# IK2277/ultimate-tictactoe-alphazero

Measured on NVIDIA B200. Metric: self-play moves/sec (50 sims/move), higher is better.
Workload: dtype bf16

## Files before the change

### ultimate-tictactoe-alphazero_b200/csrc/common.cuh

```cuda
#pragma once
#include <cuda_bf16.h>
#include <cuda_runtime.h>
#include <stdint.h>
#include <stdio.h>

#include "../../include/uttt_b200.h"
#include "uttt_rules.cuh"

namespace uttt {

void set_error(const char* fmt, ...);

#define UTTT_CUDA_OK(expr)                                                                   \
    do {                                                                                     \
        cudaError_t _e = (expr);                                                             \
        if (_e != cudaSuccess) {                                                             \
            ::uttt::set_error("%s failed: %s (%s:%d)", #expr, cudaGetErrorString(_e), __FILE__, __LINE__); \
            return 1;                                                                        \
        }                                                                                    \
    } while (0)

#define UTTT_CHECK(cond, ...)               \
    do {                                    \
        if (!(cond)) {                      \
            ::uttt::set_error(__VA_ARGS__); \
            return 2;                       \
        }                                   \
    } while (0)

static inline int ceil_div(int64_t a, int64_t b) { return (int)((a + b - 1) / b); }

#ifdef __CUDACC__
__device__ __forceinline__ void pdl_wait() { asm volatile("griddepcontrol.wait;" ::: "memory"); }
__device__ __forceinline__ void pdl_trigger() { asm volatile("griddepcontrol.launch_dependents;" ::: "memory"); }
template <typename... KArgs, typename... Args>
cudaError_t launch_pdl(void (*kernel)(KArgs...), dim3 grid, dim3 block, size_t smem, cudaStream_t s, Args... args) {
    cudaLaunchConfig_t cfg = {};
    cfg.gridDim = grid; cfg.blockDim = block; cfg.dynamicSmemBytes = smem; cfg.stream = s;
    cudaLaunchAttribute attr[1];
    attr[0].id = cudaLaunchAttributeProgrammaticStreamSerialization;
    attr[0].val.programmaticStreamSerializationAllowed = 1;
    cfg.attrs = attr; cfg.numAttrs = 1;
    return cudaLaunchKernelEx(&cfg, kernel, KArgs(args)...);
}
#endif

constexpr int NET_C = 128;
constexpr int NET_BLOCKS = 16;
constexpr int NET_LAYERS = 2 * NET_BLOCKS;
// ... 43 lines not shown
    const float* value;
    int32_t row_stride, copy_stride;
    int32_t* out_counts;
    int32_t* out_n;
    uint32_t seed;
    uint64_t game0;
    int64_t n_games;
    unsigned long long* counters;
    PackedState* hist_states;
    uint16_t* hist_counts;
    uint8_t* hist_actions;
    int32_t* hist_len;
    int8_t* hist_final;
    uint8_t* slot_flags;
    unsigned long long* dbg_tree;
};

cudaError_t launch_tree_begin(const TreeParams& p, cudaStream_t s);
cudaError_t launch_tree_round(const TreeParams& p, cudaStream_t s);
cudaError_t launch_tree_tp_begin(const TreeParams& p, cudaStream_t s);
cudaError_t launch_tree_tp_round(const TreeParams& p, cudaStream_t s);
cudaError_t launch_hash_eval(const PackedState* states, const int32_t* k, const int32_t* count, int max_rows,
                             float* policy, float* value, int row_stride, int copy_stride, cudaStream_t s);
cudaError_t launch_scores(const int32_t* counts, const int32_t* n, int n_trees, float temperature,
                          float* scores, cudaStream_t s);
cudaError_t launch_dirichlet(uint32_t seed, uint64_t game0, int64_t n, int n_children, float alpha, float* out, cudaStream_t s);
cudaError_t launch_boltzman(const float* xs, int n, float temperature, float* out, cudaStream_t s);

cudaError_t launch_scan_lens(const int32_t* lens, int64_t n, int64_t* offsets, cudaStream_t s);
cudaError_t launch_pack_samples(const PackedState* states, const uint16_t* counts, const int32_t* lens, const int8_t* final_lose,
                                const int64_t* offsets, int64_t n_games, void* out, int64_t cap_samples, cudaStream_t s);
cudaError_t launch_unpack_samples(const void* samples, int64_t n, float* x, float* policy, float* value, cudaStream_t s);

// ... 34 lines not shown
                              float* out, cudaStream_t s);
cudaError_t launch_trunk_fp32(const NetWeights& w, const __nv_bfloat16* planes, const int32_t* count, int max_rows,
                              float* act_a, float* act_b, cudaStream_t s);
cudaError_t launch_heads_fc(const NetWeights& w, const float* headfeat, const int32_t* count, int max_rows, float* policy,
                            float* value, int row_stride, cudaStream_t s);
cudaError_t launch_heads(const NetWeights& w, const float* act_f32, const __nv_bfloat16* act_bf16,
                         const int32_t* count, int max_rows, float* policy, float* value, int row_stride,
                         cudaStream_t s);
cudaError_t launch_trunk_x3(const NetWeights& w, const __nv_bfloat16* planes, float* headfeat, const int32_t* count,
                            int max_rows, float* skip, int n_sm, cudaStream_t s, long long* dbg);
int trunk_pp_cap1(int n_sm);
cudaError_t launch_trunk_pp_large(const NetWeights& w, const __nv_bfloat16* planes, float* headfeat, const int32_t* count,
                                  int max_rows, float* skip, int n_sm, cudaStream_t s, long long* dbg);
cudaError_t launch_trunk_auto(const NetWeights& w, const __nv_bfloat16* planes, float* headfeat, const int32_t* count, int max_rows,
                              float* skip, int n_sm, cudaStream_t s, long long* dbg, float* policy, float* value,
                              const uint8_t* slot_flags = nullptr, int n_slots = 0);

}
```

### ultimate-tictactoe-alphazero_b200/csrc/engine.cu

```cuda
#include <math.h>
#include <stdlib.h>
#include <string.h>

#include <vector>

#include "common.cuh"

using namespace uttt;

namespace {

constexpr int CHECK_EVERY = 8;
constexpr int N_LANES = 2;
constexpr int N_WINDOWS = 2;
constexpr int EV_POOL = N_WINDOWS * CHECK_EVERY * 4 * N_LANES;

__global__ void set_int_kernel(int32_t* p, int32_t v) { *p = v; }
__global__ void set_u64_kernel(unsigned long long* p, unsigned long long v) { *p = v; }

template <typename T>
cudaError_t dmalloc(T** p, size_t n) { return cudaMalloc((void**)p, n * sizeof(T)); }

}

// ... 94 lines not shown
    bool heads_fused = false;
    if (evaluator == UTTT_EVAL_NET_FP32) {
        if (ev3) cudaEventRecord(ev3[0], s);
        UTTT_CUDA_OK(launch_trunk_fp32(e->w, b.nn_planes, count, max_rows, b.act_a, b.act_b, s));
        e->prof_launches[1] += 1 + 2 * NET_BLOCKS;
    } else if (evaluator == UTTT_EVAL_NET_BF16X3) {
        if (ev3) cudaEventRecord(ev3[0], s);
        UTTT_CUDA_OK(launch_trunk_x3(e->w, b.nn_planes, b.headfeat, count, max_rows, b.resid, e->n_sm, s, e->tc_dbg));
        e->prof_launches[1] += 1;
    } else if (evaluator == UTTT_EVAL_NET_BF16) {
        if (ev3) cudaEventRecord(ev3[0], s);
        heads_fused = max_rows <= trunk_pp_cap1(e->n_sm);
        UTTT_CHECK(heads_fused || !b.slot_flags, "slot mode needs the fused heads");
        UTTT_CUDA_OK(launch_trunk_auto(e->w, b.nn_planes, b.headfeat, count, max_rows, b.resid, e->n_sm, s, e->tc_dbg,
                                       heads_fused ? b.policy : nullptr, heads_fused ? b.value : nullptr, b.slot_flags,
                                       b.n_slots));
        if (!heads_fused)
            UTTT_CUDA_OK(launch_trunk_pp_large(e->w, b.nn_planes, b.headfeat, count, max_rows, b.resid, e->n_sm, s, e->tc_dbg));
        e->prof_launches[1] += 1;
    } else {
        UTTT_CHECK(false, "evaluator %d cannot run on the device", evaluator);
    }
    if (ev3) cudaEventRecord(ev3[1], s);
    if (heads_fused) {
        if (ev3 && e->prof_level >= 2) cudaEventRecord(ev3[2], s);
        return 0;
    }
    if (evaluator == UTTT_EVAL_NET_BF16 || evaluator == UTTT_EVAL_NET_BF16X3)
        UTTT_CUDA_OK(launch_heads_fc(e->w, b.headfeat, count, max_rows, b.policy, b.value, 1, s));
    else
        UTTT_CUDA_OK(launch_heads(e->w, b.act_a, nullptr, count, max_rows, b.policy, b.value, 1, s));
// ... 69 lines not shown
    uttt_engine* e = new uttt_engine();
    memset(&e->tp, 0, sizeof(e->tp));
    memset(&e->w, 0, sizeof(e->w));
    e->cfg = *cfg;
    e->trace_on = false;
    e->progress_cb = nullptr;
    e->progress_user = nullptr;
    e->prof_level = getenv("UTTT_PROFILE") ? atoi(getenv("UTTT_PROFILE")) : 1;
    e->prof_sample = getenv("UTTT_PROFILE_SAMPLE") ? atoi(getenv("UTTT_PROFILE_SAMPLE")) : 4;
    if (e->prof_sample < 1) e->prof_sample = 1;
    e->lane_threshold = getenv("UTTT_LANE_THRESHOLD") ? atoi(getenv("UTTT_LANE_THRESHOLD")) : 1024;
    UTTT_CUDA_OK(net_fp32_init());
    UTTT_CUDA_OK(trunk_tc2_init());
    UTTT_CUDA_OK(trunk_pp_init());
    UTTT_CUDA_OK(trunk_auto_init());
    cudaDeviceProp prop;
    UTTT_CUDA_OK(cudaGetDeviceProperties(&prop, cfg->device));
    e->n_sm = prop.multiProcessorCount;
    e->node_cap = 1 + 81 + 81 * cfg->max_sims;
    e->rows_per_slot = cfg->max_batch < TP_MAX_LEAVES ? cfg->max_batch : TP_MAX_LEAVES;
    UTTT_CUDA_OK(cudaStreamCreateWithFlags(&e->stream, cudaStreamNonBlocking));
    size_t S = (size_t)cfg->n_slots, NC = (size_t)e->node_cap, G = (size_t)cfg->max_games;
    size_t R = S * (size_t)e->rows_per_slot;
    TreeParams& t = e->tp;
    t.node_cap = e->node_cap;
    if (ealloc(e, &t.root, S) || ealloc(e, &t.leaf_state, S * TP_MAX_LEAVES) ||
        ealloc(e, &t.tp_paths, S * TP_MAX_LEAVES * PATH_CAP) || ealloc(e, &t.tp_aux, S * 2 * TP_MAX_LEAVES) || ealloc(e, &t.ctl, S) ||
        ealloc(e, &t.path, S * PATH_CAP) || ealloc(e, &t.nodes, S * NC) ||
        ealloc(e, &t.nn_states, R) || ealloc(e, &t.nn_planes, R * 243 + 8) || ealloc(e, &t.nn_tree, R) ||
        ealloc(e, &t.nn_k, R) || ealloc(e, &t.nn_count, 2 * N_LANES) || ealloc(e, &t.out_counts, S * 81) ||
// ... 16 lines not shown
        for (int w = 0; w < N_WINDOWS; w++) UTTT_CUDA_OK(cudaEventCreateWithFlags(&e->ev_win[w][i], cudaEventDisableTiming));
    }
    UTTT_CUDA_OK(cudaEventCreateWithFlags(&e->ev_fork, cudaEventDisableTiming));
    UTTT_CUDA_OK(cudaEventCreateWithFlags(&e->ev_fwd, cudaEventDisableTiming));
    UTTT_CUDA_OK(cudaEventCreateWithFlags(&e->ev_idle, cudaEventDisableTiming));
    e->fwd_pending = false;
    UTTT_CUDA_OK(cudaMallocHost((void**)&e->h_counters, 8 * (1 + N_WINDOWS) * sizeof(unsigned long long)));
    UTTT_CUDA_OK(cudaMallocHost((void**)&e->h_count, 2 * sizeof(int32_t)));
    for (int i = 0; i < EV_POOL; i++) UTTT_CUDA_OK(cudaEventCreate(&e->ev[i]));
    t.policy = e->policy;
    t.value = e->value;
    t.dbg_tree = nullptr;
    if (getenv("UTTT_DEBUG_TREE")) {
        if (ealloc(e, &t.dbg_tree, 48)) { uttt_destroy(e); return 1; }
        UTTT_CUDA_OK(cudaMemset(t.dbg_tree, 0, 48 * sizeof(unsigned long long)));
    }
    t.max_terminal = getenv("UTTT_MAX_TERMINAL") ? atoi(getenv("UTTT_MAX_TERMINAL")) : 4;
    t.dir_alpha = 0.3f;
    t.dir_eps = 0.25f;
    t.temperature = 1.0f;
    *out = e;
    return 0;
}

int uttt_destroy(uttt_engine* e) {
    if (!e) return 0;
    cudaSetDevice(e->cfg.device);
    cudaDeviceSynchronize();
    for (void* p : e->allocs) cudaFree(p);
    release_weights(e->w);
// ... 450 lines not shown
                0ll, d[1] - d[0], d[2] - d[0], d[3] - d[0], d[4] - d[0], d[5] - d[0], d[6] - d[0], d[8] - d[0], d[9] - d[0], d[10] - d[0], d[11] - d[0],
                d[12] - d[0], d[13] - d[0], d[14] - d[0]);
        fprintf(stderr, "tc2 detail, layer 20 -> 21 (cycles rel. accumulator observed by epilogue thread 0): last MMA of layer 20 committed %lld | "
                "first chunk loaded %lld, stored %lld, fenced %lld, chunks published %lld %lld %lld %lld | issuer of tile 0 passed the "
                "act barrier of quarter 0..3 at %lld %lld %lld %lld\n", d[12] - d[0], d[1] - d[0], d[2] - d[0], d[3] - d[0], d[4] - d[0],
                d[5] - d[0], d[6] - d[0], d[7] - d[0], d[8] - d[0], d[9] - d[0], d[10] - d[0], d[11] - d[0]);
        long long au[10];
        UTTT_CUDA_OK(cudaMemcpy(au, e->tc_dbg + 200, sizeof(au), cudaMemcpyDeviceToHost));
        fprintf(stderr, "heads FC tail (cycles rel. body done): barriers ready %lld, features loaded %lld, chunk 0/1/2 landed %lld %lld %lld, "
                "policy FC done %lld, all FC done %lld, exit %lld\n", au[3] - au[1], au[4] - au[1], au[5] - au[1], au[6] - au[1],
                au[7] - au[1], au[8] - au[1], au[9] - au[1], au[2] - au[1]);
        fprintf(stderr, "trunk_auto_kernel CTA 0 (cycles rel. entry): body done %lld, heads FC done %lld (warp 0's exit; heads = %lld)\n",
                au[1] - au[0], au[2] - au[0], au[2] - au[1]);
        fprintf(stderr, "trunk phases (cycles rel. entry): setup %lld, first MMA %lld, last epilogue %lld, exit %lld\n", ph[1] - ph[0],
                (long long)out128[0] - ph[0], ph[2] - ph[0], ph[3] - ph[0]);
    }
    return 0;
}

int uttt_debug_batch_histogram(uttt_engine* e, int64_t* out64, int32_t reset) {
    UTTT_CHECK(e && out64, "null argument");
    UTTT_CUDA_OK(cudaSetDevice(e->cfg.device));
    UTTT_CUDA_OK(cudaDeviceSynchronize());
    UTTT_CUDA_OK(cudaMemcpy(out64, e->tc_dbg + 128, 64 * sizeof(long long), cudaMemcpyDeviceToHost));
    if (reset) UTTT_CUDA_OK(cudaMemset(e->tc_dbg + 128, 0, 64 * sizeof(long long)));
    return 0;
}

int uttt_debug_trace(uttt_engine* e, int enable) {
    UTTT_CHECK(e != nullptr, "null engine");
// ... 51 lines not shown
```

### ultimate-tictactoe-alphazero_b200/csrc/net_auto.cu

```cuda
#include "heads_fc.cuh"
#include "net_pp_kernel.cuh"
#include "net_tc2_kernel.cuh"

namespace uttt {

static_assert(tc2::Cfg<>::THREADS == pp::THREADS, "one block size for both bodies");
constexpr int AUTO_SMEM = tc2::Cfg<>::SMEM_BYTES > pp::Cfg<1>::SMEM_BYTES ? tc2::Cfg<>::SMEM_BYTES : pp::Cfg<1>::SMEM_BYTES;
static_assert(HEADS_SMEM_BYTES <= AUTO_SMEM, "the fused heads reuse the trunk's shared memory");

constexpr int SLOT_CHUNKS = 17;
__device__ __forceinline__ void scan_slots(const uint8_t* __restrict__ flags, int n_slots, int n_pairs, int pair, int small_cap,
                                           int* s_npos, int* s_src) {
    const int lane = threadIdx.x & 31;
    uint32_t mine = 0;
#pragma unroll
    for (int j = 0; j < SLOT_CHUNKS; j++) {
        const int idx = lane + 32 * j;
        if (idx < n_slots && flags[idx]) mine |= 1u << j;
    }
    uint32_t bal[SLOT_CHUNKS];
    int n_pos = 0;
#pragma unroll
    for (int j = 0; j < SLOT_CHUNKS; j++) {
        bal[j] = __ballot_sync(0xFFFFFFFFu, (mine >> j) & 1u);
// ... 2 lines not shown
    const int P = n_pos <= small_cap ? tc2::group_positions(n_pos, n_pairs) : pp::pair_positions<1>(n_pos, n_pairs);
    const int first = pair * P, last = min(n_pos, first + P);
    int run = 0;
#pragma unroll
    for (int j = 0; j < SLOT_CHUNKS; j++) {
        if ((bal[j] >> lane) & 1u) {
            const int rank = run + __popc(bal[j] & ((1u << lane) - 1u));
            if (rank >= first && rank < last) s_src[rank - first] = lane + 32 * j;
        }
        run += __popc(bal[j]);
    }
    if (lane == 0) *s_npos = n_pos;
}

constexpr int AUTO_SMEM_TOTAL = AUTO_SMEM + 64;

__global__ void __cluster_dims__(2, 1, 1) __launch_bounds__(pp::THREADS, 1)
trunk_auto_kernel(const __nv_bfloat16* __restrict__ res_w8, const __nv_bfloat16* __restrict__ conv_in_w8,
                  const __nv_bfloat16* __restrict__ res_w18, const __nv_bfloat16* __restrict__ conv_in_w18,
                  const __nv_bfloat16* __restrict__ bias_2sm,
                  const __nv_bfloat16* __restrict__ planes, const float* __restrict__ headw, float* headfeat, uint4* skip,
                  const int32_t* __restrict__ count, int small_cap, int cap1, long long* dbg,
                  HeadsFC fc, float* policy, float* value ,
                  const uint8_t* __restrict__ slot_flags, int n_slots ) {
    extern __shared__ __align__(1024) uint8_t smem[];
    pdl_trigger();
    pdl_wait();
    const bool stamp = dbg && blockIdx.x == 0 && threadIdx.x == 0;
    if (stamp) dbg[200] = clock64();
    const int n_pairs = (int)gridDim.x >> 1, pair = (int)blockIdx.x >> 1;
    int* s_src = reinterpret_cast<int*>(smem + AUTO_SMEM);
    int* s_npos = s_src + 8;
    int n_pos;
    if (slot_flags) {
        if (threadIdx.x < 32) scan_slots(slot_flags, n_slots, n_pairs, pair, small_cap, s_npos, s_src);
        __syncthreads();
        n_pos = *s_npos;
    } else {
        n_pos = *count;
    }
    const int* src = slot_flags ? s_src : nullptr;
    const bool small = n_pos <= small_cap;
    if (n_pos <= 0 || n_pos > cap1) return;
    tcx::count_batch(dbg, n_pos);
    if (!small)
        pp::trunk_pp_body<1>(res_w18, conv_in_w18, bias_2sm, planes, headw, headfeat, skip, dbg, n_pos, src);
    else
        tc2::trunk_tc2_body<false>(res_w8, conv_in_w8, bias_2sm, planes, headw, headfeat, skip, dbg, n_pos, src, 0, false);
    if (stamp) dbg[201] = clock64();
    if (policy == nullptr) return;
    const int P = small ? tc2::group_positions(n_pos, n_pairs) : pp::pair_positions<1>(n_pos, n_pairs);
    const int first = pair * P, last = min(n_pos, first + P);
    const int rank = (int)tcx::cluster_rank();
    const int row0 = first + rank;
    const int np = row0 < last ? (last - row0 + 1) >> 1 : 0;
    static_assert((pp::Cfg<1>::MAX_PA + pp::Cfg<1>::MAX_PB + 1) / 2 <= HEADS_P, "one heads call per CTA");
    if (np == 0) return;
    heads_fc_block(fc, headfeat, row0, 2, np, policy, value, 1, reinterpret_cast<float*>(smem), stamp ? dbg + 203 : nullptr,
                   src ? src + rank : nullptr);
    if (stamp) dbg[202] = clock64();
}

cudaError_t trunk_auto_init() {
    return cudaFuncSetAttribute(trunk_auto_kernel, cudaFuncAttributeMaxDynamicSharedMemorySize, AUTO_SMEM_TOTAL);
}

cudaError_t launch_trunk_auto(const NetWeights& w, const __nv_bfloat16* planes, float* headfeat, const int32_t* count, int max_rows,
                              float* skip, int n_sm, cudaStream_t s, long long* dbg, float* policy, float* value,
                              const uint8_t* slot_flags, int n_slots) {
    int pairs = n_sm / 2;
    if (max_rows < pairs) pairs = max_rows < 1 ? 1 : max_rows;
    const int small_cap = (n_sm / 2) * tc2::Cfg<>::MAX_P;
    const int cap1 = (n_sm / 2) * (pp::Cfg<1>::MAX_PA + pp::Cfg<1>::MAX_PB);
    if (policy && max_rows > cap1) return cudaErrorInvalidValue;
    if (slot_flags && (!policy || n_slots > 32 * SLOT_CHUNKS || n_slots > max_rows)) return cudaErrorInvalidValue;
    return launch_pdl(trunk_auto_kernel, dim3(2 * pairs), dim3(pp::THREADS), AUTO_SMEM_TOTAL, s, w.res_w_2sm, w.conv_in_w_2sm,
                      w.res_w_2sm18, w.conv_in_w_2sm18, w.bias_blk_2sm, planes, w.head_w, headfeat, reinterpret_cast<uint4*>(skip),
                      count, small_cap, cap1, dbg, heads_fc_of(w), policy, value, slot_flags, n_slots);
}

}
```

### ultimate-tictactoe-alphazero_b200/csrc/net_pp_kernel.cuh

```cuda
#pragma once
#include "tc_common.cuh"

namespace uttt {
namespace pp {

using namespace tcx;

constexpr int POS_ROWS = 100;
constexpr int LEAD = 11;
constexpr int LT = 2;
constexpr int NG = 2;
constexpr int BIAS_BYTES = 2048;
constexpr int CONST_BYTES = 4096;
constexpr int EPI_WARPS = 8 * LT;
constexpr int THREADS = (EPI_WARPS + 1 + LT) * 32;
constexpr int SKIP_ROWS = 128 * LT;
constexpr int GROUP_LAYERS = NET_LAYERS + 1;
constexpr uint32_t IDESC = IDESC_M256_N128_BF16;
constexpr int a_rows(int tiles) { return (LEAD + 128 * tiles + 11 + 7) / 8 * 8; }

template <int LTB>
struct Cfg {
    static constexpr int MAX_PA = 5, MAX_PB = (LTB == 1) ? 2 : 5;
    static constexpr int PANEL_A = a_rows(LT) * 16, PANEL_B = a_rows(LTB) * 16;
// ... 37 lines not shown
__host__ __device__ inline int pair_positions(int n_pos, int n_pairs) {
    int P = (n_pos + n_pairs - 1) / n_pairs;
    return P < 1 ? 1 : (P > Cfg<LTB>::MAX_PA + Cfg<LTB>::MAX_PB ? Cfg<LTB>::MAX_PA + Cfg<LTB>::MAX_PB : P);
}

template <int LTB>
__device__ __forceinline__ void trunk_pp_body(const __nv_bfloat16* __restrict__ wq,
                const __nv_bfloat16* __restrict__ wq_in,
                const __nv_bfloat16* __restrict__ wq_bias,
                const __nv_bfloat16* __restrict__ planes,
                const float* __restrict__ headw,
                float* headfeat,
                uint4* skip,
                long long* dbg,
                int n_pos,
                const int* src_rows) {
    using C = Cfg<LTB>;
    constexpr int STAGES = C::STAGES, BAR_OFF = C::BAR_OFF, HEAD_OFF = C::HEAD_OFF, CONST_OFF = C::CONST_OFF,
                  STAGE_BLOCKS = C::STAGE_BLOCKS, STAGE_BYTES = C::STAGE_BYTES, STAGES_PER_LAYER = C::STAGES_PER_LAYER,
                  IN_STAGES = C::IN_STAGES;
    constexpr int MAX_P = C::MAX_PA;
    extern __shared__ __align__(1024) uint8_t smem[];
    const int warp = threadIdx.x >> 5, lane = threadIdx.x & 31;
    const uint32_t rank = cluster_rank();
    const uint32_t peer = rank ^ 1u;
    const int n_pairs = (int)gridDim.x >> 1, pair = (int)blockIdx.x >> 1;
    const int Ptot = pair_positions<LTB>(n_pos, n_pairs);
    const int n_super = (n_pos + Ptot - 1) / Ptot;
    if (pair >= n_super) return;
    const int PA = Ptot < MAX_P ? Ptot : MAX_P;
    const Geo geo[NG] = {make_geo(PA, rank), make_geo(Ptot - PA, rank)};
    const bool any_tiles = geo[0].T0 + geo[1].T0 > 0;

    uint8_t* sA = smem;
    const uint32_t sA_u = smem_u32(sA);
    const uint32_t sB_u = sA_u + C::W_OFF;
    auto grp_off = [](int g) { return (uint32_t)(g == 0 ? 0 : C::A_BYTES); };
    auto grp_panel = [](int g) { return (uint32_t)(g == 0 ? C::PANEL_A : C::PANEL_B); };
    const uint32_t bar_u = sA_u + BAR_OFF;
    const uint32_t bar_full = bar_u, bar_empty = bar_u + 8 * STAGES, bar_grp = bar_u + 16 * STAGES;
    constexpr int GRP_BARS = 2 * LT;
    auto bar_accum = [&](int g, int t) { return bar_grp + 8u * (uint32_t)(g * GRP_BARS + t); };
    auto bar_act = [&](int g, int t) { return bar_grp + 8u * (uint32_t)(g * GRP_BARS + LT + t); };
    static_assert(16 * STAGES + 8 * NG * GRP_BARS + 4 <= 512, "barrier block");
    uint32_t* tmem_holder = reinterpret_cast<uint32_t*>(smem + BAR_OFF + 16 * STAGES + 8 * NG * GRP_BARS);
    const int bnd_quarter = (rank == 0) ? 3 : 0;

    if (threadIdx.x == 0) {
        for (int i = 0; i < STAGES; i++) {
            mbar_init(bar_full + 8 * i, rank == 0 ? 2 : 1);
            mbar_init(bar_empty + 8 * i, LT);
        }
        for (int g = 0; g < NG; g++) {
            for (int t = 0; t < LT; t++) {
                mbar_init(bar_accum(g, t), 1);
                mbar_init(bar_act(g, t), 8 + (t > 0 ? 2 : 0) + (t < geo[g].tiles - 1 ? 2 : 0) + ((rank == 0 && t < geo[g].T1) ? 1 : 0));
            }
        }
        asm volatile("fence.mbarrier_init.release.cluster;" ::: "memory");
    }
    if (warp == EPI_WARPS + 1) {
        asm volatile("tcgen05.alloc.cta_group::2.sync.aligned.shared::cta.b32 [%0], %1;" ::"r"(smem_u32(tmem_holder)), "r"(512u)
                     : "memory");
        asm volatile("tcgen05.relinquish_alloc_permit.cta_group::2.sync.aligned;" ::: "memory");
    }
    for (int i = threadIdx.x; i < (C::A_BYTES + C::B_BYTES) / 16; i += THREADS) reinterpret_cast<uint4*>(sA)[i] = make_uint4(0, 0, 0, 0);
    for (int i = threadIdx.x; i < CONST_BYTES / 16; i += THREADS)
        reinterpret_cast<uint4*>(sA + CONST_OFF)[i] = (i < 128) ? make_uint4(0x3F803F80u, 0, 0, 0) : make_uint4(0, 0, 0, 0);
    fence_async_smem();
    tc_fence_before();
    __syncthreads();
    cluster_sync_all();
    tc_fence_after();
    const uint32_t tmem_base = *tmem_holder;

    int iter = 0;
    for (int sg = pair; sg < n_super; sg += n_pairs, iter++) {
        if (warp < EPI_WARPS) {
            const int lt = warp >> 3, quarter = warp & 3, chalf = (warp >> 2) & 1;
            const int lr = lt * 128 + quarter * 32 + lane;
            const uint4 zero4 = make_uint4(0, 0, 0, 0);
// ... 301 lines not shown
                                    if (dbg && blockIdx.x == 0 && iter == 0 && lt == 0 && layer < 16) dbg[(16 * g + layer) * 4 + 1] = clock64();
                                }
                            }
                            advance();
                        }
                    }
                }
            }
            __syncwarp();
        }
    }

    tc_fence_before();
    __syncthreads();
    cluster_sync_all();
    if (warp == EPI_WARPS + 1) {
        asm volatile("tcgen05.dealloc.cta_group::2.sync.aligned.b32 %0, %1;" ::"r"(tmem_base), "r"(512u) : "memory");
    }
}

}
}
```

### ultimate-tictactoe-alphazero_b200/csrc/net_tc2_kernel.cuh

```cuda
#pragma once
#include <stdlib.h>

#include "tc_common.cuh"


namespace uttt {
namespace tc2 {

constexpr int POS_ROWS = 100;
constexpr int LEAD = 11;
constexpr int GROUP_LAYERS = NET_LAYERS + 1;

template <bool X3 = false>
struct Cfg {
    static constexpr int LOC_TILES = 2;
    static constexpr int MAX_P = 5;
    static constexpr int AROWS = (LEAD + 128 * LOC_TILES + 11 + 7) / 8 * 8;
    static constexpr int PANEL_BYTES = AROWS * 16;
    static constexpr int ACT_PANELS = X3 ? 32 : 16;
    static constexpr int A_BYTES = (ACT_PANELS + 2) * PANEL_BYTES;
    static constexpr int STAGES = X3 ? 3 : 8;
    static constexpr int STAGE_BLOCKS = X3 ? 6 : 8;
    static constexpr int NCO = 64;
    static constexpr int SUB_BYTES = 2 * NCO * 16;
// ... 24 lines not shown
    if (P == 4) P = 5;
    return P;
}

template <bool X3>
__device__ __forceinline__ void trunk_tc2_body(const __nv_bfloat16* __restrict__ wq,
                 const __nv_bfloat16* __restrict__ wq_in,
                 const __nv_bfloat16* __restrict__ wq_bias,
                 const __nv_bfloat16* __restrict__ planes,
                 const float* __restrict__ headw,
                 float* headfeat,
                 uint4* skip,
                 long long* dbg,
                 int n_pos,
                 const int* src_rows,
                 int pos_base, bool solo) {
    using C = Cfg<X3>;
    constexpr int LOC_TILES = C::LOC_TILES, PANEL_BYTES = C::PANEL_BYTES, A_BYTES = C::A_BYTES,
                  STAGES = C::STAGES, BAR_OFF = C::BAR_OFF, EPI_WARPS = C::EPI_WARPS, THREADS = C::THREADS,
                  SKIP_ROWS = C::SKIP_ROWS, NQ = C::NQ, STAGE_BLOCKS = C::STAGE_BLOCKS, STAGE_BYTES = C::STAGE_BYTES,
                  STAGES_PER_LAYER = C::STAGES_PER_LAYER, IN_STAGES = C::IN_STAGES, GROUP_STAGES = C::GROUP_STAGES,
                  ACT_PANELS = C::ACT_PANELS, SKIP_U4 = C::SKIP_U4, BLOCK_BYTES = C::BLOCK_BYTES;
    extern __shared__ __align__(1024) uint8_t smem[];
    const long long t_entry = clock64();
    const int warp = threadIdx.x >> 5, lane = threadIdx.x & 31;
    const uint32_t rank = cluster_rank();
    const int n_pairs = solo ? 1 : (int)gridDim.x >> 1, pair = solo ? 0 : (int)blockIdx.x >> 1;
    const int P = group_positions(n_pos, n_pairs);
    const int T = (P * POS_ROWS + 127) / 128;
    const int T0 = (T + 1) >> 1;
    const int tiles = (rank == 0) ? T0 : T - T0;
    const int tile0 = (rank == 0) ? 0 : T0;
    const int n_groups = (n_pos + P - 1) / P;
    if (pair >= n_groups) return;
    const int T1 = T - T0;
    const bool has_peer = T1 > 0;

    uint8_t* sA = smem;
    const uint32_t sA_u = smem_u32(sA);
    const uint32_t sB_u = sA_u + A_BYTES;
    const uint32_t bar_u = sA_u + BAR_OFF;
    const uint32_t bar_full = bar_u, bar_empty = bar_u + 8 * STAGES, bar_accum = bar_u + 16 * STAGES,
                   bar_act = bar_accum + 8 * LOC_TILES;
    constexpr int N_BARS = 2 * STAGES + LOC_TILES * (1 + NQ);
    static_assert(8 * N_BARS + 4 <= 256, "barrier block");
    uint32_t* tmem_holder = reinterpret_cast<uint32_t*>(smem + BAR_OFF + 8 * N_BARS);
    const int bnd_tile = (rank == 0) ? tiles - 1 : 0;
    const int bnd_quarter = (rank == 0) ? 3 : 0;

    if (threadIdx.x == 0) {
        for (int i = 0; i < STAGES; i++) {
            mbar_init(bar_full + 8 * i, rank == 0 ? 2 : 1);
            mbar_init(bar_empty + 8 * i, T0);
        }
        for (int t = 0; t < LOC_TILES; t++) {
            mbar_init(bar_accum + 8 * t, 1);
            int c = 8 + (t > 0 ? 2 : 0) + (t < tiles - 1 ? 2 : 0);
            if (rank == 0 && t < T1) c += 1;
            for (int q = 0; q < NQ; q++) mbar_init(bar_act + 8 * (t * NQ + q), c);
        }
        asm volatile("fence.mbarrier_init.release.cluster;" ::: "memory");
    }
    if (warp == EPI_WARPS + 1) {
        asm volatile("tcgen05.alloc.cta_group::2.sync.aligned.shared::cta.b32 [%0], %1;" ::"r"(smem_u32(tmem_holder)),
                     "r"(C::TMEM_COLS)
                     : "memory");
        if (!solo) asm volatile("tcgen05.relinquish_alloc_permit.cta_group::2.sync.aligned;" ::: "memory");
    }
    for (int i = threadIdx.x; i < A_BYTES / 16; i += THREADS) reinterpret_cast<uint4*>(sA)[i] = make_uint4(0, 0, 0, 0);
    __syncthreads();
    for (int i = threadIdx.x; i < C::AROWS; i += THREADS)
        reinterpret_cast<uint4*>(sA + (size_t)ACT_PANELS * PANEL_BYTES)[i] = make_uint4(0x3F803F80u, X3 ? 0x00003F80u : 0u, 0, 0);
    fence_async_all();
    tc_fence_before();
    __syncthreads();
    cluster_sync_all();
    tc_fence_after();
    const uint32_t tmem_base = *tmem_holder;
    const uint32_t peer = rank ^ 1u;
    if (dbg && blockIdx.x == 0 && threadIdx.x == 0) { dbg[192] = t_entry; dbg[193] = clock64(); }

    int iter = 0;
    for (int g = pair; g < n_groups; g += n_pairs, iter++) {
        if (warp < EPI_WARPS) {
// ... 303 lines not shown
                                if (dbg && blockIdx.x == 0 && iter == 0 && lt == 0 && layer == 20) dbg[172] = clock64();
                            }
                        }
                        advance();
                    }
                }
            }
            __syncwarp();
        }
    }

    if (dbg && blockIdx.x == 0 && threadIdx.x == 0) dbg[194] = clock64();
    tc_fence_before();
    __syncthreads();
    cluster_sync_all();
    if (warp == EPI_WARPS + 1)
        asm volatile("tcgen05.dealloc.cta_group::2.sync.aligned.b32 %0, %1;" ::"r"(tmem_base), "r"(C::TMEM_COLS) : "memory");
    if (solo && threadIdx.x == 0) {
#pragma unroll
        for (int i = 0; i < N_BARS; i++) asm volatile("mbarrier.inval.shared::cta.b64 [%0];" ::"r"(bar_u + 8 * i) : "memory");
    }
    if (dbg && blockIdx.x == 0 && threadIdx.x == 0) dbg[195] = clock64();
}

}
}
```

### ultimate-tictactoe-alphazero_b200/csrc/tree_kernels.cu

```cuda
#include "tree_common.cuh"

namespace uttt {

__device__ void init_root(const TreeParams& P, const TreeView& T, TreeCtl& c, const PackedState& rs, int lane) {
    uint32_t lm[3];
    int L = legal_mask(rs, lm);
    if (P.flags & UTTT_SP_PYSEARCH) {
        if (lane == 0) T.node[0] = make_uint4(0x7Fu << 16, 0u, 0u, 0u);
        c.n_nodes = 1;
        c.n_root = L;
        c.sims_left = P.sims;
        c.path_len = 0;
        c.pend_k = 0;
        return;
    }
    float pu = (L > 0) ? __fdiv_rn(1.0f, (float)L) : 0.0f;
    if (lane == 0) T.node[0] = make_uint4(0x7Fu << 16, 0u, 0u, (L > 0 ? 1u : 0u) | ((uint32_t)L << 20));
    for (int a = lane; a < 81; a += 32)
        if (legal_bit(lm, a)) T.node[1 + legal_rank(lm, a)] = make_node(a, pu);
    c.n_nodes = 1 + L;
    c.n_root = L;
    c.sims_left = P.sims;
    c.path_len = 0;
    c.pend_k = 0;
// ... 151 lines not shown
        init_state(rs);
        warp_store_state(P.root + t, rs, lane);
    } else {
        rs = warp_load_state(P.root + t, lane);
    }
    init_root(P, T, c, rs, lane);
    if (c.n_root == 0) {
        c.phase = PHASE_DONE;
        if (lane == 0) { P.out_n[t] = 0; atomicAdd(P.counters + 6, 1ull); }
    } else {
        c.phase = PHASE_SEARCH;
    }
    if (lane == 0) P.ctl[t] = c;
}

__global__ void __launch_bounds__(32 * WARPS_PER_BLOCK) tree_round_kernel(TreeParams P) {
    pdl_trigger();
    pdl_wait();
    int t = blockIdx.x * WARPS_PER_BLOCK + (threadIdx.x >> 5);
    int lane = threadIdx.x & 31;
    if (blockIdx.x == 0 && threadIdx.x == 0) P.nn_count[P.parity ^ 1] = 0;
    if (t >= P.n_trees) return;
    const long long t_start = P.dbg_tree ? clock64() : 0;
    int dbg_moved = 0;
    const uint32_t leaf_raw = warp_load_state_issue(P.leaf_state + t, lane);
    const uint32_t root_raw = warp_load_state_issue(P.root + t, lane);
    TreeCtl c = P.ctl[t];
    if (c.phase == PHASE_DONE) return;
    TreeView T = view_of(P, t);

    if (c.phase == PHASE_PENDING) {
        if (P.flags & UTTT_SP_PYSEARCH) apply_leaf_py(P, T, c, warp_load_state_finish(leaf_raw), lane);
        else apply_leaf(P, T, c, warp_load_state_finish(leaf_raw), lane);
        if (c.phase == PHASE_DONE) {
            if (lane == 0) { P.ctl[t] = c; if (P.slot_flags) P.slot_flags[t] = 0; }
            return;
        }
// ... 129 lines not shown
        c.nn_row = row;
        c.path_len = plen;
        break;
    }
    if (lane == 0) {
        P.ctl[t] = c;
        if (P.slot_flags) P.slot_flags[t] = (c.phase == PHASE_PENDING) ? 1 : 0;
    }
    if (P.dbg_tree && lane == 0) {
        unsigned long long dt = (unsigned long long)(clock64() - t_start);
        unsigned long long* d = P.dbg_tree + 3 * (min(n_terminal, 7) + dbg_moved);
        atomicAdd(d, dt); atomicAdd(d + 1, 1ull); atomicMax(d + 2, dt);
    }
}

__global__ void __launch_bounds__(128) hash_eval_kernel(const PackedState* __restrict__ states,
                                                        const int32_t* __restrict__ kk,
                                                        const int32_t* __restrict__ count, float* __restrict__ policy,
                                                        float* __restrict__ value, int row_stride, int copy_stride) {
    int row = blockIdx.x * 4 + (threadIdx.x >> 5);
    int lane = threadIdx.x & 31;
    if (row >= *count) return;
    PackedState st = warp_load_state(states + row, lane);
    uint32_t h = state_hash(st);
    int copies = (copy_stride == 0) ? 1 : kk[row];
    for (int c = 0; c < copies; c++) {
        size_t r = (size_t)row * row_stride + (size_t)c * copy_stride;
        for (int a = lane; a < 81; a += 32) {
            float num = (float)((mix32(h + (uint32_t)a) & 0xFFFFu) + 1u);
            policy[r * 81 + a] = __fdiv_rn(__fdiv_rn(num, 65536.0f), 81.0f);
// ... 29 lines not shown
    for (int i = n; i < 81; i++) s[i] = 0.0f;
}

__global__ void boltzman_kernel(const float* __restrict__ xs, int n, float temperature, float* __restrict__ out) {
    if (blockIdx.x != 0 || threadIdx.x != 0) return;
    float inv = __fdiv_rn(1.0f, temperature), sum = 0.0f;
    for (int i = 0; i < n; i++) {
        float v = (inv == 1.0f) ? xs[i] : powf(xs[i], inv);
        out[i] = v;
        sum = __fadd_rn(sum, v);
    }
    if (sum > 0.0f)
        for (int i = 0; i < n; i++) out[i] = __fdiv_rn(out[i], sum);
}

cudaError_t launch_tree_begin(const TreeParams& p, cudaStream_t s) {
    tree_begin_kernel<<<ceil_div(p.n_trees, WARPS_PER_BLOCK), 32 * WARPS_PER_BLOCK, 0, s>>>(p);
    return cudaGetLastError();
}
cudaError_t launch_tree_round(const TreeParams& p, cudaStream_t s) {
    return launch_pdl(tree_round_kernel, dim3(ceil_div(p.n_trees, WARPS_PER_BLOCK)), dim3(32 * WARPS_PER_BLOCK), 0, s, p);
}
cudaError_t launch_hash_eval(const PackedState* states, const int32_t* k, const int32_t* count, int max_rows,
                             float* policy, float* value, int row_stride, int copy_stride, cudaStream_t s) {
    hash_eval_kernel<<<ceil_div(max_rows, 4), 128, 0, s>>>(states, k, count, policy, value, row_stride, copy_stride);
    return cudaGetLastError();
}
cudaError_t launch_scores(const int32_t* counts, const int32_t* n, int n_trees, float temperature, float* scores,
                          cudaStream_t s) {
    scores_kernel<<<ceil_div(n_trees, 128), 128, 0, s>>>(counts, n, n_trees, temperature, scores);
// ... 9 lines not shown
```

### ultimate-tictactoe-alphazero_b200/csrc/tree_tp_kernels.cu

```cuda
#include "tree_common.cuh"

namespace uttt {

constexpr uint32_t LINK_PENDING = 0xFFFFFu;

__device__ __forceinline__ float u01(uint32_t x) { return ((float)(x >> 8) + 0.5f) * (1.0f / 16777216.0f); }

__device__ float gamma_sample(float alpha, uint32_t seed, uint64_t game, uint32_t ply, uint32_t child) {
    float a = alpha < 1.0f ? alpha + 1.0f : alpha;
    float d = a - 1.0f / 3.0f, c = rsqrtf(9.0f * d);
    float g = d;
    for (uint32_t attempt = 0; attempt < 64; attempt++) {
        Philox4 r = philox4x32(seed, 3u, (uint32_t)game, (uint32_t)(game >> 32) ^ (ply << 16), child, attempt);
        float u1 = u01(r.x), u2 = u01(r.y), u3 = u01(r.z);
        float x = sqrtf(-2.0f * logf(u1)) * cosf(6.283185307f * u2);
        float v = 1.0f + c * x;
        if (v <= 0.0f) continue;
        v = v * v * v;
        if (logf(u3) < 0.5f * x * x + d - d * v + d * logf(v)) { g = d * v; break; }
    }
    if (alpha < 1.0f) {
        Philox4 r = philox4x32(seed, 3u, (uint32_t)game, (uint32_t)(game >> 32) ^ (ply << 16), child, 0xFFFFu);
        g *= powf(u01(r.w), 1.0f / alpha);
    }
// ... 288 lines not shown
        }
        if (terminals) {
            c.sims_left -= terminals;
            if (lane == 0) atomicAdd(P.counters + 3, (unsigned long long)terminals);
        }
        if (got > 0) {
            c.pend_k = got;
            c.phase = PHASE_PENDING;
            break;
        }
        if (c.sims_left > 0) break;
    }
    if (lane == 0) P.ctl[t] = c;
}

cudaError_t launch_tree_tp_begin(const TreeParams& p, cudaStream_t s) {
    tree_tp_begin_kernel<<<ceil_div(p.n_trees, WARPS_PER_BLOCK), 32 * WARPS_PER_BLOCK, 0, s>>>(p);
    return cudaGetLastError();
}
cudaError_t launch_tree_tp_round(const TreeParams& p, cudaStream_t s) {
    tree_tp_round_kernel<<<ceil_div(p.n_trees, WARPS_PER_BLOCK), 32 * WARPS_PER_BLOCK, 0, s>>>(p);
    return cudaGetLastError();
}

}
```

Before: 182,400.

## Hoist TMEM alloc and smem zeroing before PDL wait to overlap tree kernel

The trunk kernel now allocates TMEM and zeroes its shared-memory operand buffers before griddepcontrol.wait, so this setup overlaps the tail of the preceding tree-round grid. The shared carveout of the tree kernels is set to max-shared and their registers are capped with __maxnreg__, so trunk CTAs can become resident alongside tree blocks. Optional globaltimer probes record how often setup finishes before the tree grid ends. The risks are register spills from the new caps and contention for SM resources while both grids are resident.

```diff
diff --git a/ultimate-tictactoe-alphazero_b200/csrc/common.cuh b/ultimate-tictactoe-alphazero_b200/csrc/common.cuh
--- a/ultimate-tictactoe-alphazero_b200/csrc/common.cuh
+++ b/ultimate-tictactoe-alphazero_b200/csrc/common.cuh
@@ -33,6 +33,11 @@
 #ifdef __CUDACC__
 __device__ __forceinline__ void pdl_wait() { asm volatile("griddepcontrol.wait;" ::: "memory"); }
 __device__ __forceinline__ void pdl_trigger() { asm volatile("griddepcontrol.launch_dependents;" ::: "memory"); }
+__device__ __forceinline__ unsigned long long globaltimer_ns() {
+    unsigned long long t;
+    asm volatile("mov.u64 %0, %%globaltimer;" : "=l"(t));
+    return t;
+}
 template <typename... KArgs, typename... Args>
 cudaError_t launch_pdl(void (*kernel)(KArgs...), dim3 grid, dim3 block, size_t smem, cudaStream_t s, Args... args) {
     cudaLaunchConfig_t cfg = {};
@@ -106,9 +111,12 @@
     int8_t* hist_final;
     uint8_t* slot_flags;
     unsigned long long* dbg_tree;
+    unsigned long long* dbg_phase;
 };
 
 cudaError_t launch_tree_begin(const TreeParams& p, cudaStream_t s);
+cudaError_t tree_init();
+cudaError_t tree_tp_init();
 cudaError_t launch_tree_round(const TreeParams& p, cudaStream_t s);
 cudaError_t launch_tree_tp_begin(const TreeParams& p, cudaStream_t s);
 cudaError_t launch_tree_tp_round(const TreeParams& p, cudaStream_t s);
@@ -173,6 +181,6 @@
                                   int max_rows, float* skip, int n_sm, cudaStream_t s, long long* dbg);
 cudaError_t launch_trunk_auto(const NetWeights& w, const __nv_bfloat16* planes, float* headfeat, const int32_t* count, int max_rows,
                               float* skip, int n_sm, cudaStream_t s, long long* dbg, float* policy, float* value,
-                              const uint8_t* slot_flags = nullptr, int n_slots = 0);
+                              const uint8_t* slot_flags = nullptr, int n_slots = 0, unsigned long long* phase = nullptr);
 
 }
diff --git a/ultimate-tictactoe-alphazero_b200/csrc/engine.cu b/ultimate-tictactoe-alphazero_b200/csrc/engine.cu
--- a/ultimate-tictactoe-alphazero_b200/csrc/engine.cu
+++ b/ultimate-tictactoe-alphazero_b200/csrc/engine.cu
@@ -132,7 +132,7 @@
         UTTT_CHECK(heads_fused || !b.slot_flags, "slot mode needs the fused heads");
         UTTT_CUDA_OK(launch_trunk_auto(e->w, b.nn_planes, b.headfeat, count, max_rows, b.resid, e->n_sm, s, e->tc_dbg,
                                        heads_fused ? b.policy : nullptr, heads_fused ? b.value : nullptr, b.slot_flags,
-                                       b.n_slots));
+                                       b.n_slots, e->tp.dbg_phase));
         if (!heads_fused)
             UTTT_CUDA_OK(launch_trunk_pp_large(e->w, b.nn_planes, b.headfeat, count, max_rows, b.resid, e->n_sm, s, e->tc_dbg));
         e->prof_launches[1] += 1;
@@ -232,6 +232,8 @@
     UTTT_CUDA_OK(trunk_tc2_init());
     UTTT_CUDA_OK(trunk_pp_init());
     UTTT_CUDA_OK(trunk_auto_init());
+    UTTT_CUDA_OK(tree_init());
+    UTTT_CUDA_OK(tree_tp_init());
     cudaDeviceProp prop;
     UTTT_CUDA_OK(cudaGetDeviceProperties(&prop, cfg->device));
     e->n_sm = prop.multiProcessorCount;
@@ -278,6 +280,11 @@
     if (getenv("UTTT_DEBUG_TREE")) {
         if (ealloc(e, &t.dbg_tree, 48)) { uttt_destroy(e); return 1; }
         UTTT_CUDA_OK(cudaMemset(t.dbg_tree, 0, 48 * sizeof(unsigned long long)));
+    }
+    t.dbg_phase = nullptr;
+    if (getenv("UTTT_DEBUG_PHASES")) {
+        if (ealloc(e, &t.dbg_phase, 8)) { uttt_destroy(e); return 1; }
+        UTTT_CUDA_OK(cudaMemset(t.dbg_phase, 0, 8 * sizeof(unsigned long long)));
     }
     t.max_terminal = getenv("UTTT_MAX_TERMINAL") ? atoi(getenv("UTTT_MAX_TERMINAL")) : 4;
     t.dir_alpha = 0.3f;
@@ -758,6 +765,15 @@
                 au[1] - au[0], au[2] - au[0], au[2] - au[1]);
         fprintf(stderr, "trunk phases (cycles rel. entry): setup %lld, first MMA %lld, last epilogue %lld, exit %lld\n", ph[1] - ph[0],
                 (long long)out128[0] - ph[0], ph[2] - ph[0], ph[3] - ph[0]);
+        if (e->tp.dbg_phase) {
+            unsigned long long r[5];
+            UTTT_CUDA_OK(cudaMemcpy(r, e->tp.dbg_phase, sizeof(r), cudaMemcpyDeviceToHost));
+            UTTT_CUDA_OK(cudaMemset(e->tp.dbg_phase + 1, 0, 4 * sizeof(unsigned long long)));
+            const double n = r[1] ? (double)r[1] : 1.0;
+            fprintf(stderr, "trunk_auto_kernel residency: %llu CTA launches, %llu (%.1f %%) with their set-up done before the tree grid "
+                    "ended (by %.2f us on average), mean wait %.2f us\n", r[1], r[2], 100.0 * r[2] / n, r[2] ? 1e-3 * r[3] / r[2] : 0.0,
+                    1e-3 * r[4] / n);
+        }
     }
     return 0;
 }
diff --git a/ultimate-tictactoe-alphazero_b200/csrc/net_auto.cu b/ultimate-tictactoe-alphazero_b200/csrc/net_auto.cu
--- a/ultimate-tictactoe-alphazero_b200/csrc/net_auto.cu
+++ b/ultimate-tictactoe-alphazero_b200/csrc/net_auto.cu
@@ -40,23 +40,52 @@
 }
 
 constexpr int AUTO_SMEM_TOTAL = AUTO_SMEM + 64;
+constexpr int AUTO_ZERO_BYTES = tc2::Cfg<>::A_BYTES > pp::Cfg<1>::A_BYTES + pp::Cfg<1>::B_BYTES ? tc2::Cfg<>::A_BYTES
+                                                                                                 : pp::Cfg<1>::A_BYTES + pp::Cfg<1>::B_BYTES;
+static_assert(tc2::Cfg<>::TMEM_COLS == 512u, "both bodies use all 512 TMEM columns");
 
-__global__ void __cluster_dims__(2, 1, 1) __launch_bounds__(pp::THREADS, 1)
+__global__ void __cluster_dims__(2, 1, 1) __maxnreg__(88)
 trunk_auto_kernel(const __nv_bfloat16* __restrict__ res_w8, const __nv_bfloat16* __restrict__ conv_in_w8,
                   const __nv_bfloat16* __restrict__ res_w18, const __nv_bfloat16* __restrict__ conv_in_w18,
                   const __nv_bfloat16* __restrict__ bias_2sm,
                   const __nv_bfloat16* __restrict__ planes, const float* __restrict__ headw, float* headfeat, uint4* skip,
                   const int32_t* __restrict__ count, int small_cap, int cap1, long long* dbg,
                   HeadsFC fc, float* policy, float* value ,
-                  const uint8_t* __restrict__ slot_flags, int n_slots ) {
+                  const uint8_t* __restrict__ slot_flags, int n_slots ,
+                  unsigned long long* phase ) {
     extern __shared__ __align__(1024) uint8_t smem[];
     pdl_trigger();
+    const int warp = threadIdx.x >> 5;
+    int* s_src = reinterpret_cast<int*>(smem + AUTO_SMEM);
+    int* s_npos = s_src + 8;
+    uint32_t* s_tmem = reinterpret_cast<uint32_t*>(s_src + 9);
+    if (warp == pp::EPI_WARPS + 1) {
+        asm volatile("tcgen05.alloc.cta_group::2.sync.aligned.shared::cta.b32 [%0], %1;" ::"r"(tcx::smem_u32(s_tmem)), "r"(512u)
+                     : "memory");
+        asm volatile("tcgen05.relinquish_alloc_permit.cta_group::2.sync.aligned;" ::: "memory");
+    }
+    for (int i = threadIdx.x; i < AUTO_ZERO_BYTES / 16; i += pp::THREADS) reinterpret_cast<uint4*>(smem)[i] = make_uint4(0, 0, 0, 0);
+    tcx::tc_fence_before();
+    __syncthreads();
+    tcx::tc_fence_after();
+    const unsigned long long t_wait = phase ? globaltimer_ns() : 0ull;
     pdl_wait();
+    if (phase && threadIdx.x == 0) {
+        const unsigned long long t_tree = *reinterpret_cast<volatile unsigned long long*>(phase);
+        atomicAdd(phase + 1, 1ull);
+        atomicAdd(phase + 4, globaltimer_ns() - t_wait);
+        if (t_wait < t_tree) { atomicAdd(phase + 2, 1ull); atomicAdd(phase + 3, t_tree - t_wait); }
+    }
+    auto free_tmem = [&]() {
+        tcx::tc_fence_before();
+        __syncthreads();
+        tcx::tc_fence_after();
+        if (warp == pp::EPI_WARPS + 1)
+            asm volatile("tcgen05.dealloc.cta_group::2.sync.aligned.b32 %0, %1;" ::"r"(*s_tmem), "r"(512u) : "memory");
+    };
     const bool stamp = dbg && blockIdx.x == 0 && threadIdx.x == 0;
     if (stamp) dbg[200] = clock64();
     const int n_pairs = (int)gridDim.x >> 1, pair = (int)blockIdx.x >> 1;
-    int* s_src = reinterpret_cast<int*>(smem + AUTO_SMEM);
-    int* s_npos = s_src + 8;
     int n_pos;
     if (slot_flags) {
         if (threadIdx.x < 32) scan_slots(slot_flags, n_slots, n_pairs, pair, small_cap, s_npos, s_src);
@@ -67,12 +96,13 @@
     }
     const int* src = slot_flags ? s_src : nullptr;
     const bool small = n_pos <= small_cap;
-    if (n_pos <= 0 || n_pos > cap1) return;
+    if (n_pos <= 0 || n_pos > cap1) { free_tmem(); return; }
     tcx::count_batch(dbg, n_pos);
     if (!small)
-        pp::trunk_pp_body<1>(res_w18, conv_in_w18, bias_2sm, planes, headw, headfeat, skip, dbg, n_pos, src);
+        pp::trunk_pp_body<1>(res_w18, conv_in_w18, bias_2sm, planes, headw, headfeat, skip, dbg, n_pos, src, s_tmem);
     else
-        tc2::trunk_tc2_body<false>(res_w8, conv_in_w8, bias_2sm, planes, headw, headfeat, skip, dbg, n_pos, src, 0, false);
+        tc2::trunk_tc2_body<false>(res_w8, conv_in_w8, bias_2sm, planes, headw, headfeat, skip, dbg, n_pos, src, 0, false, s_tmem);
+    free_tmem();
     if (stamp) dbg[201] = clock64();
     if (policy == nullptr) return;
     const int P = small ? tc2::group_positions(n_pos, n_pairs) : pp::pair_positions<1>(n_pos, n_pairs);
@@ -93,7 +123,7 @@
 
 cudaError_t launch_trunk_auto(const NetWeights& w, const __nv_bfloat16* planes, float* headfeat, const int32_t* count, int max_rows,
                               float* skip, int n_sm, cudaStream_t s, long long* dbg, float* policy, float* value,
-                              const uint8_t* slot_flags, int n_slots) {
+                              const uint8_t* slot_flags, int n_slots, unsigned long long* phase) {
     int pairs = n_sm / 2;
     if (max_rows < pairs) pairs = max_rows < 1 ? 1 : max_rows;
     const int small_cap = (n_sm / 2) * tc2::Cfg<>::MAX_P;
@@ -102,7 +132,7 @@
     if (slot_flags && (!policy || n_slots > 32 * SLOT_CHUNKS || n_slots > max_rows)) return cudaErrorInvalidValue;
     return launch_pdl(trunk_auto_kernel, dim3(2 * pairs), dim3(pp::THREADS), AUTO_SMEM_TOTAL, s, w.res_w_2sm, w.conv_in_w_2sm,
                       w.res_w_2sm18, w.conv_in_w_2sm18, w.bias_blk_2sm, planes, w.head_w, headfeat, reinterpret_cast<uint4*>(skip),
-                      count, small_cap, cap1, dbg, heads_fc_of(w), policy, value, slot_flags, n_slots);
+                      count, small_cap, cap1, dbg, heads_fc_of(w), policy, value, slot_flags, n_slots, phase);
 }
 
 }
diff --git a/ultimate-tictactoe-alphazero_b200/csrc/net_pp_kernel.cuh b/ultimate-tictactoe-alphazero_b200/csrc/net_pp_kernel.cuh
--- a/ultimate-tictactoe-alphazero_b200/csrc/net_pp_kernel.cuh
+++ b/ultimate-tictactoe-alphazero_b200/csrc/net_pp_kernel.cuh
@@ -75,7 +75,8 @@
                 uint4* skip,
                 long long* dbg,
                 int n_pos,
-                const int* src_rows) {
+                const int* src_rows,
+                uint32_t* pre_tmem = nullptr) {
     using C = Cfg<LTB>;
     constexpr int STAGES = C::STAGES, BAR_OFF = C::BAR_OFF, HEAD_OFF = C::HEAD_OFF, CONST_OFF = C::CONST_OFF,
                   STAGE_BLOCKS = C::STAGE_BLOCKS, STAGE_BYTES = C::STAGE_BYTES, STAGES_PER_LAYER = C::STAGES_PER_LAYER,
@@ -104,7 +105,7 @@
     auto bar_accum = [&](int g, int t) { return bar_grp + 8u * (uint32_t)(g * GRP_BARS + t); };
     auto bar_act = [&](int g, int t) { return bar_grp + 8u * (uint32_t)(g * GRP_BARS + LT + t); };
     static_assert(16 * STAGES + 8 * NG * GRP_BARS + 4 <= 512, "barrier block");
-    uint32_t* tmem_holder = reinterpret_cast<uint32_t*>(smem + BAR_OFF + 16 * STAGES + 8 * NG * GRP_BARS);
+    uint32_t* tmem_holder = pre_tmem ? pre_tmem : reinterpret_cast<uint32_t*>(smem + BAR_OFF + 16 * STAGES + 8 * NG * GRP_BARS);
     const int bnd_quarter = (rank == 0) ? 3 : 0;
 
     if (threadIdx.x == 0) {
@@ -120,12 +121,14 @@
         }
         asm volatile("fence.mbarrier_init.release.cluster;" ::: "memory");
     }
-    if (warp == EPI_WARPS + 1) {
-        asm volatile("tcgen05.alloc.cta_group::2.sync.aligned.shared::cta.b32 [%0], %1;" ::"r"(smem_u32(tmem_holder)), "r"(512u)
-                     : "memory");
-        asm volatile("tcgen05.relinquish_alloc_permit.cta_group::2.sync.aligned;" ::: "memory");
+    if (!pre_tmem) {
+        if (warp == EPI_WARPS + 1) {
+            asm volatile("tcgen05.alloc.cta_group::2.sync.aligned.shared::cta.b32 [%0], %1;" ::"r"(smem_u32(tmem_holder)), "r"(512u)
+                         : "memory");
+            asm volatile("tcgen05.relinquish_alloc_permit.cta_group::2.sync.aligned;" ::: "memory");
+        }
+        for (int i = threadIdx.x; i < (C::A_BYTES + C::B_BYTES) / 16; i += THREADS) reinterpret_cast<uint4*>(sA)[i] = make_uint4(0, 0, 0, 0);
     }
-    for (int i = threadIdx.x; i < (C::A_BYTES + C::B_BYTES) / 16; i += THREADS) reinterpret_cast<uint4*>(sA)[i] = make_uint4(0, 0, 0, 0);
     for (int i = threadIdx.x; i < CONST_BYTES / 16; i += THREADS)
         reinterpret_cast<uint4*>(sA + CONST_OFF)[i] = (i < 128) ? make_uint4(0x3F803F80u, 0, 0, 0) : make_uint4(0, 0, 0, 0);
     fence_async_smem();
@@ -457,7 +460,7 @@
     tc_fence_before();
     __syncthreads();
     cluster_sync_all();
-    if (warp == EPI_WARPS + 1) {
+    if (!pre_tmem && warp == EPI_WARPS + 1) {
         asm volatile("tcgen05.dealloc.cta_group::2.sync.aligned.b32 %0, %1;" ::"r"(tmem_base), "r"(512u) : "memory");
     }
 }
diff --git a/ultimate-tictactoe-alphazero_b200/csrc/net_tc2_kernel.cuh b/ultimate-tictactoe-alphazero_b200/csrc/net_tc2_kernel.cuh
--- a/ultimate-tictactoe-alphazero_b200/csrc/net_tc2_kernel.cuh
+++ b/ultimate-tictactoe-alphazero_b200/csrc/net_tc2_kernel.cuh
@@ -62,7 +62,8 @@
                  long long* dbg,
                  int n_pos,
                  const int* src_rows,
-                 int pos_base, bool solo) {
+                 int pos_base, bool solo,
+                 uint32_t* pre_tmem = nullptr) {
     using C = Cfg<X3>;
     constexpr int LOC_TILES = C::LOC_TILES, PANEL_BYTES = C::PANEL_BYTES, A_BYTES = C::A_BYTES,
                   STAGES = C::STAGES, BAR_OFF = C::BAR_OFF, EPI_WARPS = C::EPI_WARPS, THREADS = C::THREADS,
@@ -92,7 +93,7 @@
                    bar_act = bar_accum + 8 * LOC_TILES;
     constexpr int N_BARS = 2 * STAGES + LOC_TILES * (1 + NQ);
     static_assert(8 * N_BARS + 4 <= 256, "barrier block");
-    uint32_t* tmem_holder = reinterpret_cast<uint32_t*>(smem + BAR_OFF + 8 * N_BARS);
+    uint32_t* tmem_holder = pre_tmem ? pre_tmem : reinterpret_cast<uint32_t*>(smem + BAR_OFF + 8 * N_BARS);
     const int bnd_tile = (rank == 0) ? tiles - 1 : 0;
     const int bnd_quarter = (rank == 0) ? 3 : 0;
 
@@ -109,13 +110,15 @@
         }
         asm volatile("fence.mbarrier_init.release.cluster;" ::: "memory");
     }
-    if (warp == EPI_WARPS + 1) {
-        asm volatile("tcgen05.alloc.cta_group::2.sync.aligned.shared::cta.b32 [%0], %1;" ::"r"(smem_u32(tmem_holder)),
-                     "r"(C::TMEM_COLS)
-                     : "memory");
-        if (!solo) asm volatile("tcgen05.relinquish_alloc_permit.cta_group::2.sync.aligned;" ::: "memory");
+    if (!pre_tmem) {
+        if (warp == EPI_WARPS + 1) {
+            asm volatile("tcgen05.alloc.cta_group::2.sync.aligned.shared::cta.b32 [%0], %1;" ::"r"(smem_u32(tmem_holder)),
+                         "r"(C::TMEM_COLS)
+                         : "memory");
+            if (!solo) asm volatile("tcgen05.relinquish_alloc_permit.cta_group::2.sync.aligned;" ::: "memory");
+        }
+        for (int i = threadIdx.x; i < A_BYTES / 16; i += THREADS) reinterpret_cast<uint4*>(sA)[i] = make_uint4(0, 0, 0, 0);
     }
-    for (int i = threadIdx.x; i < A_BYTES / 16; i += THREADS) reinterpret_cast<uint4*>(sA)[i] = make_uint4(0, 0, 0, 0);
     __syncthreads();
     for (int i = threadIdx.x; i < C::AROWS; i += THREADS)
         reinterpret_cast<uint4*>(sA + (size_t)ACT_PANELS * PANEL_BYTES)[i] = make_uint4(0x3F803F80u, X3 ? 0x00003F80u : 0u, 0, 0);
@@ -449,7 +452,7 @@
     tc_fence_before();
     __syncthreads();
     cluster_sync_all();
-    if (warp == EPI_WARPS + 1)
+    if (!pre_tmem && warp == EPI_WARPS + 1)
         asm volatile("tcgen05.dealloc.cta_group::2.sync.aligned.b32 %0, %1;" ::"r"(tmem_base), "r"(C::TMEM_COLS) : "memory");
     if (solo && threadIdx.x == 0) {
 #pragma unroll
diff --git a/ultimate-tictactoe-alphazero_b200/csrc/tree_kernels.cu b/ultimate-tictactoe-alphazero_b200/csrc/tree_kernels.cu
--- a/ultimate-tictactoe-alphazero_b200/csrc/tree_kernels.cu
+++ b/ultimate-tictactoe-alphazero_b200/csrc/tree_kernels.cu
@@ -189,13 +189,7 @@
     if (lane == 0) P.ctl[t] = c;
 }
 
-__global__ void __launch_bounds__(32 * WARPS_PER_BLOCK) tree_round_kernel(TreeParams P) {
-    pdl_trigger();
-    pdl_wait();
-    int t = blockIdx.x * WARPS_PER_BLOCK + (threadIdx.x >> 5);
-    int lane = threadIdx.x & 31;
-    if (blockIdx.x == 0 && threadIdx.x == 0) P.nn_count[P.parity ^ 1] = 0;
-    if (t >= P.n_trees) return;
+__device__ __forceinline__ void tree_round(const TreeParams& P, int t, int lane) {
     const long long t_start = P.dbg_tree ? clock64() : 0;
     int dbg_moved = 0;
     const uint32_t leaf_raw = warp_load_state_issue(P.leaf_state + t, lane);
@@ -355,6 +349,16 @@
     }
 }
 
+__global__ void __maxnreg__(72) tree_round_kernel(TreeParams P) {
+    pdl_trigger();
+    pdl_wait();
+    const int t = blockIdx.x * WARPS_PER_BLOCK + (threadIdx.x >> 5);
+    const int lane = threadIdx.x & 31;
+    if (blockIdx.x == 0 && threadIdx.x == 0) P.nn_count[P.parity ^ 1] = 0;
+    if (t < P.n_trees) tree_round(P, t, lane);
+    if (P.dbg_phase && lane == 0) atomicMax(P.dbg_phase, globaltimer_ns());
+}
+
 __global__ void __launch_bounds__(128) hash_eval_kernel(const PackedState* __restrict__ states,
                                                         const int32_t* __restrict__ kk,
                                                         const int32_t* __restrict__ count, float* __restrict__ policy,
@@ -414,6 +418,9 @@
         for (int i = 0; i < n; i++) out[i] = __fdiv_rn(out[i], sum);
 }
 
+cudaError_t tree_init() {
+    return cudaFuncSetAttribute(tree_round_kernel, cudaFuncAttributePreferredSharedMemoryCarveout, cudaSharedmemCarveoutMaxShared);
+}
 cudaError_t launch_tree_begin(const TreeParams& p, cudaStream_t s) {
     tree_begin_kernel<<<ceil_div(p.n_trees, WARPS_PER_BLOCK), 32 * WARPS_PER_BLOCK, 0, s>>>(p);
     return cudaGetLastError();
diff --git a/ultimate-tictactoe-alphazero_b200/csrc/tree_tp_kernels.cu b/ultimate-tictactoe-alphazero_b200/csrc/tree_tp_kernels.cu
--- a/ultimate-tictactoe-alphazero_b200/csrc/tree_tp_kernels.cu
+++ b/ultimate-tictactoe-alphazero_b200/csrc/tree_tp_kernels.cu
@@ -326,6 +326,9 @@
     if (lane == 0) P.ctl[t] = c;
 }
 
+cudaError_t tree_tp_init() {
+    return cudaFuncSetAttribute(tree_tp_round_kernel, cudaFuncAttributePreferredSharedMemoryCarveout, cudaSharedmemCarveoutMaxShared);
+}
 cudaError_t launch_tree_tp_begin(const TreeParams& p, cudaStream_t s) {
     tree_tp_begin_kernel<<<ceil_div(p.n_trees, WARPS_PER_BLOCK), 32 * WARPS_PER_BLOCK, 0, s>>>(p);
     return cudaGetLastError();
```

Result: no change. 182,400 (median of 6 runs) (-0.0%).
